# tomas-gr/RawNanoporeSignalCompression

Measured on AMD Instinct MI355X. Metric: MSamples/s encode+decode (1/2/4/8 GPU) at fixed ratio; % HBM roofline, higher is better.
Workload: dtype int16; 1 GPU; configs[1]: 100000 reads x 100000 int16 samples per GPU (1 chunk each), C5 encode+decode; reads_per_gpu=100000, samples_per_read=100000, global_reads=100000, parallelism=dp1 (reads round-robin, no data-path collective)

## Files before the change

rawnanoporesignalcompression_amd/csrc/model_capi.hip:

```cpp
#include <stdlib.h>
#include <string.h>

#define PGN_SELECT_HOST_ONLY
#include "pgn_segment.h"
#include "pgn_select.h"
#include "pgn_stitch.h"
#include "zstd1_dec.h"
#include "zstd1_model.h"

using namespace pgn::z1;

extern "C" {

size_t z1m_compress(const uint8_t* src, size_t n, uint8_t* dst, size_t cap)
{
    if (n > 0xFFFFFFF0ull || cap < compress_bound(n)) return 0;
    uint32_t* ht = (uint32_t*)calloc((size_t)1 << 15, 4);
    size_t ns = kMaxSrc / 4 + 2;
    Seq* seqs = (Seq*)malloc(ns * sizeof(Seq));
    uint8_t* codes = (uint8_t*)malloc(3 * ns);
    uint8_t* litbuf = (uint8_t*)malloc(kMaxSrc + 1);
    CompressWork* w = (CompressWork*)malloc(sizeof(CompressWork));
    size_t r = compress_serial(dst, src, n, ht, seqs, codes, codes + ns, codes + 2 * ns, litbuf, *w);
    free(w); free(litbuf); free(codes); free(seqs); free(ht);
// ... 140 lines not shown
    for (;; k++) {
        if (k % 64 == 0 && 2 * (k + 64) > maxKeys) { ok = 0; break; }
        const long pk = (long)e - 256;
        e += e >> 7;
        if (!(pk + 1 < ilimit)) break;
        const uint64_t v8 = rd64(src + pk);
        if (rd32(src + pk + 1) == (uint32_t)(v8 >> 16)) { ok = 0; break; }
        const uint32_t keys[2] = {(uint32_t)v8 ^ (hash_word(v8, p.hashLog, p.mls) * 0x9E3779B1u),
                                  (uint32_t)(v8 >> 8) ^ (hash_word(v8 >> 8, p.hashLog, p.mls) * 0x9E3779B1u)};
        for (int j = 0; j < 2 && ok; j++) {
            const uint32_t a = cert_fmix32(keys[j]), b = cert_fmix32(keys[j] ^ 0x5BD1E995u);
            const uint64_t m = (1ull << (a & 63u)) | (1ull << ((a >> 6) & 63u)) | (1ull << ((a >> 12) & 63u)) |
                               (1ull << ((a >> 18) & 63u)) | (1ull << ((a >> 24) & 63u)) | (1ull << (b & 63u));
            uint64_t* w = filt + ((b >> 6) & (words - 1));
            if ((*w & m) == m) ok = 0;
            *w |= m;
        }
        if (!ok) break;
    }
    free(filt);
    return ok;
}

long z1m_decompress(const uint8_t* src, size_t n, uint8_t* dst, size_t cap)
{
    DecWork* w = (DecWork*)malloc(sizeof(DecWork));
    long r = decompress_frames(src, n, dst, cap, *w);
    free(w);
    return r;
}

unsigned z1m_huf_lengths(const uint32_t* count, unsigned maxSymbolValue, uint8_t* nbBits)
{
    HufNode* nodes = (HufNode*)calloc(1024, sizeof(HufNode));
    huf_sort_serial(nodes + 1, count, maxSymbolValue);
    uint16_t val[256];
    const unsigned r = huf_build_from_sorted(nodes, maxSymbolValue, 11, nbBits, val);
    free(nodes);
    return r;
}

long long z1m_content_size(const uint8_t* src, size_t n)
{
    bool ok = false;
    uint64_t v = frame_content_size(src, n, &ok);
    return ok ? (long long)v : -1;
// ... 80 lines not shown
```

rawnanoporesignalcompression_amd/csrc/pgn_kernels.hip:

```cpp
#include <hip/hip_runtime.h>
#include <stdio.h>
#include <stdlib.h>
#include <string.h>

#include <algorithm>
#include <condition_variable>
#include <mutex>
#include <vector>

#include "../../include/pgnano_hip.h"
#include "../../include/pgnano_pod5.h"
#include "pgn_c5.h"
#include "pgn_internal.h"
#include "pgn_segment.h"
#include "pgn_stitch.h"
#include "pgn_ctc.h"
#include "pgn_crf.h"
#include "pgn_crf_post.h"
#include "pgn_qual.h"
#include "pgn_select.h"
#include "pgn_vbz.h"
#include "pgn_variants.h"
#include "pgn_zdec.h"
#include "pgn_zenc.h"
// ... 215 lines not shown
        sz[4] = tL;
    }
}

constexpr size_t kSplitWgMaxChunks = 64;

__global__ __launch_bounds__(64) __attribute__((amdgpu_waves_per_eu(4))) void enc_zstd_kernel(EncArgs a)
{
    const int lane = lane_id();
    const EncLayout lay = enc_layout();
    uint8_t* sbase = a.slotScratch + (size_t)blockIdx.x * a.slotBytes;
    EncScratch S;
    S.ht = (uint32_t*)(sbase + lay.ht);
    S.seqs = (z1::Seq*)(sbase + lay.seqs);
    S.codes = sbase + lay.codes;
    S.lit = sbase + lay.lit;
    S.seqSection = sbase + lay.seqSection;
    S.seqWork = (z1::SeqWork*)(sbase + lay.seqWork);
    S.maxSeq = kMaxEncSeq;
    S.huf = (uint32_t*)(sbase + lay.huf);
    S.coop = nullptr;
    uint32_t epoch = a.epochs[blockIdx.x];
    PhaseProf P;
    P.init(a.prof);
    const size_t G = a.G, units = (size_t)a.nu * G;
    while (true) {
        uint32_t u = 0;
        if (lane == 0) u = atomicAdd(a.queue, 1u);
        u = __builtin_amdgcn_readfirstlane(u);
        if (u >= units) break;
        const int s = a.nu == 1 ? 0 : unit_stream((uint32_t)(u / G));
        const size_t g = u % G;
        if (a.base + g >= a.nchunks) continue;
        const uint32_t n = a.sizes[g * kStreams + s];
        if (a.sizes[g * kStreams] == ~0u) continue;
        ht_next_epoch(S.ht, epoch, n);
        const uint8_t* src = a.streams + g * kChunkStreamBytes + (a.nu == 1 ? a.sizes[g * kStreams + 1] : stream_off(s));
        uint8_t* dst = a.frames + g * kChunkFrameBytes + frame_off(s);
        const size_t fsz = zstd1_compress_wave(dst, src, n, S, epoch & 0xFFu, P);
        if (lane == 0) a.fsizes[g * kStreams + s] = (uint32_t)fsz;
        wave_sync();
    }
    if (lane == 0) a.epochs[blockIdx.x] = epoch;
    P.flush();
}

__device__ __noinline__ void enc_place_frame(const EncArgs& a, size_t g, int s, const uint8_t* fr, uint32_t f)
// ... 42 lines not shown
    if (a.base + g >= a.nchunks) return;
    if (a.sizes[g * kStreams] == ~0u) return;
    __shared__ uint32_t winAll[(kCoopEncWaves - 1) * kWinWords];
    __shared__ CoopEncCmd cmdLds;
    lds_enc_cmd* cmd = (lds_enc_cmd*)&cmdLds;
    if (wid != 0) {
        coop_enc_helper_wave(wid, cmd, (lds_u32*)&winAll[(wid - 1) * kWinWords]);
        return;
    }
    const EncLayout lay = enc_layout();
    uint8_t* sbase = a.slotScratch + (size_t)u * a.slotBytes;
    EncScratch S;
    S.ht = (uint32_t*)(sbase + lay.ht);
    S.seqs = (z1::Seq*)(sbase + lay.seqs);
    S.codes = sbase + lay.codes;
    S.lit = sbase + lay.lit;
    S.seqSection = sbase + lay.seqSection;
    S.seqWork = (z1::SeqWork*)(sbase + lay.seqWork);
    S.maxSeq = kMaxEncSeq;
    S.huf = (uint32_t*)(sbase + lay.huf);
    S.coop = cmd;
    uint32_t epoch = a.epochs[u];
    PhaseProf P;
    P.init(a.prof);
    const uint32_t n = a.sizes[g * kStreams + s];
    ht_next_epoch(S.ht, epoch, n);
    const uint8_t* src = a.streams + g * kChunkStreamBytes + (a.nu == 1 ? a.sizes[g * kStreams + 1] : stream_off(s));
    uint8_t* dst = a.frames + g * kChunkFrameBytes + frame_off(s);
    const size_t fsz = zstd1_compress_wave<true>(dst, src, n, S, epoch & 0xFFu, P);
    if (lane == 0) {
        a.fsizes[g * kStreams + s] = (uint32_t)fsz;
        a.epochs[u] = epoch;
    }
    coop_enc_finish(cmd);
    if (a.lookback) enc_place_frame(a, g, s, dst, (uint32_t)fsz);
    P.flush();
}

__global__ __launch_bounds__(64) void enc_assemble_kernel(EncArgs a)
{
    const size_t g = blockIdx.x;
    const size_t c = a.base + g;
    if (g >= a.G || c >= a.nchunks) return;
    const int lane = lane_id();
    const uint32_t* sz = a.sizes + g * kStreams;
    if (sz[0] == ~0u) return;
    PhaseProf P;
// ... 998 lines not shown
template <int Codec>
__global__ __launch_bounds__(64) __attribute__((amdgpu_waves_per_eu(5))) void enc_chunk_kernel(EncArgs a)
{
    constexpr int nf = codec_frames(Codec);
    constexpr bool oneFrame = nf == 1;
    const int lane = lane_id();
    const EncLayout lay = enc_layout();
    uint8_t* sbase = a.slotScratch + (size_t)blockIdx.x * a.slotBytes;
    EncScratch S;
    S.ht = (uint32_t*)(sbase + lay.ht);
    S.seqs = (z1::Seq*)(sbase + lay.seqs);
    S.codes = sbase + lay.codes;
    S.lit = sbase + lay.lit;
    S.seqSection = sbase + lay.seqSection;
    S.seqWork = (z1::SeqWork*)(sbase + lay.seqWork);
    S.maxSeq = kMaxEncSeq;
    S.huf = (uint32_t*)(sbase + lay.huf);
    S.coop = nullptr;
    const uint32_t capN = a.capN;
    uint8_t* streams = sbase + lay.bytes;
    uint8_t* fbuf = streams + chunk_stream_bytes(capN);
    uint32_t epoch = a.epochs[blockIdx.x];
    PhaseProf P;
    P.init(a.prof);
    while (true) {
        uint32_t u = 0;
        if (lane == 0) u = atomicAdd(a.queue, 1u);
        u = __builtin_amdgcn_readfirstlane(u);
        if (u >= a.nchunks) break;
        const size_t c = a.list ? a.list[u] : u;
        const uint32_t n = a.sampleCounts[c];
        if (n > capN) {
            enc_fail_chunk(a, c, PGN_ERR_UNSUPPORTED);
            continue;
        }
        const int16_t* x = a.samples + a.sampleOffsets[c];
        uint32_t sz[kStreams] = {0, 0, 0, 0, 0};
        const uint8_t* src[kStreams] = {streams, streams, streams, streams, streams};
        if (Codec == kCodecVbz || Codec == kCodecC1) {
            const uint32_t pad = (16u - (svb_key_length(n) & 15u)) & 15u;
            const uint32_t m = vbz_split_chunk(x, n, streams + pad);
            src[0] = streams + pad;
            if (Codec == kCodecVbz) {
                sz[0] = m;
            } else {
                sz[0] = n ? svb_key_length(n) : 0u;
                sz[1] = m - sz[0];
// ... 2618 lines not shown
```

rawnanoporesignalcompression_amd/csrc/pgn_wave.h:

```cpp
#pragma once
#include <hip/hip_runtime.h>
#include <stdint.h>

namespace pgn {

constexpr size_t kCodecLdsBytes = 8192;
typedef __attribute__((address_space(3))) uint32_t lds_u32;
static __shared__ __attribute__((aligned(16))) uint8_t sCodecLds[kCodecLdsBytes];

constexpr int kWave = 64;

__device__ __forceinline__ int lane_id() { return (int)__lane_id(); }

__device__ __forceinline__ uint32_t readlane_u32(uint32_t v, int l)
{
    return (uint32_t)__builtin_amdgcn_readlane((int)v, l);
}
__device__ __forceinline__ uint64_t readlane_u64(uint64_t v, int l)
{
    uint32_t lo = readlane_u32((uint32_t)v, l), hi = readlane_u32((uint32_t)(v >> 32), l);
    return ((uint64_t)hi << 32) | lo;
}
__device__ __forceinline__ uint64_t ballot(bool p) { return __ballot(p); }

// ... 154 lines not shown
        gst<uint4>(dst + i + 3072, d);
    }
    for (; i + 16 <= n; i += 1024) gst<uint4>(dst + i, gld<uint4>(src + i));
    for (size_t b = (n & ~(size_t)15) + (size_t)lane; b < n; b += 64) gst<uint8_t>(dst + b, gb(src + b));
}
__device__ inline void wave_copy8(uint8_t* dst, const uint8_t* src, size_t n)
{
    const size_t l16 = (size_t)lane_id() * 16;
    size_t base = 0;
    for (; base + 8192 <= n; base += 8192) {
        uint4 v[8];
#pragma unroll
        for (int k = 0; k < 8; k++) v[k] = gld<uint4>(src + base + l16 + 1024 * k);
#pragma unroll
        for (int k = 0; k < 8; k++) gst<uint4>(dst + base + l16 + 1024 * k, v[k]);
    }
    wave_copy(dst + base, src + base, n - base);
}
__device__ inline void wave_fill(uint8_t* dst, uint8_t v, size_t n)
{
    for (size_t i = lane_id(); i < n; i += 64) gst<uint8_t>(dst + i, v);
}

constexpr int kPhases = 16;
constexpr int kCounters = 16;
constexpr int kHufProfOff = 2 * (kPhases + kCounters);
constexpr int kProfWords = kHufProfOff + 2 * (kPhases + kCounters);
struct PhaseProf {
#ifdef PGN_PROFILE
    uint64_t* out;
    uint64_t last;
    uint64_t acc[kPhases];
    uint64_t cnt[kCounters];
    __device__ void init(uint64_t* o)
    {
        out = o;
        for (int i = 0; i < kPhases; i++) acc[i] = 0;
        for (int i = 0; i < kCounters; i++) cnt[i] = 0;
        last = o ? __builtin_amdgcn_s_memtime() : 0;
    }
    __device__ __forceinline__ void mark(int phase)
    {
        if (out) {
            uint64_t t = __builtin_amdgcn_s_memtime();
            acc[phase] += t - last;
            last = t;
        }
    }
    __device__ __forceinline__ void count(int k, uint64_t v = 1)
    {
        if (out) cnt[k] += v;
    }
    __device__ void flush()
    {
        if (out && lane_id() == 0) {
            for (int i = 0; i < kPhases; i++) atomicAdd((unsigned long long*)&out[i], (unsigned long long)acc[i]);
            for (int i = 0; i < kCounters; i++)
                atomicAdd((unsigned long long*)&out[2 * kPhases + i], (unsigned long long)cnt[i]);
        }
    }
#else
    __device__ __forceinline__ void init(uint64_t*) {}
    __device__ __forceinline__ void mark(int) {}
    __device__ __forceinline__ void count(int, uint64_t = 1) {}
    __device__ __forceinline__ void flush() {}
#endif
};

}
```

rawnanoporesignalcompression_amd/csrc/pgn_zenc.h:

```cpp
#pragma once
#ifndef PGN_AB_SKIP
#define PGN_AB_SKIP 0
#endif
#include "pgn_c5.h"
#include "pgn_wave.h"
#include "zstd1_model.h"

namespace pgn {

constexpr int kWinWords = 392;
constexpr int kFiltSlots = 512;

struct WCTable {
    uint32_t tableLog;
    uint16_t stateTable[64];
    uint32_t deltaNbBits[16];
    int32_t deltaFindState[16];
};

struct alignas(16) EncLds {
    union {
        struct {
            uint64_t filt[kFiltSlots];
            uint32_t vh0[64], vh1[64], vpk[64];
            uint32_t vd0[64], vd1[64];
        };
        struct {
            uint32_t hist2[2][256];
            union {
            uint32_t hist2x[1 + 2 * 256];
            struct {
            uint8_t nbBits[256];
            uint16_t val[256];
            union {
// ... 166 lines not shown
constexpr uint32_t kCertWords = kCodecLdsBytes / 8;
constexpr uint32_t kCertKeys = 2048;
__device__ __forceinline__ uint32_t fmix32(uint32_t x)
{
    x ^= x >> 16;
    x *= 0x85EBCA6Bu;
    x ^= x >> 13;
    x *= 0xC2B2AE35u;
    x ^= x >> 16;
    return x;
}
typedef __attribute__((address_space(3))) uint64_t lds_u64;
__device__ __forceinline__ bool cert_insert(lds_u64* words, uint32_t x)
{
    const uint32_t a = fmix32(x), b = fmix32(x ^ 0x5BD1E995u);
    const uint64_t m = (1ull << (a & 63u)) | (1ull << ((a >> 6) & 63u)) | (1ull << ((a >> 12) & 63u)) |
                       (1ull << ((a >> 18) & 63u)) | (1ull << ((a >> 24) & 63u)) | (1ull << (b & 63u));
    const uint32_t w = (b >> 6) & (kCertWords - 1u);
    const uint64_t old = __hip_atomic_fetch_or(words + w, m, __ATOMIC_RELAXED, __HIP_MEMORY_SCOPE_WORKGROUP);
    return (old & m) == m;
}
static_assert((kCertWords & (kCertWords - 1)) == 0, "filter words: a power of two");
__device__ __noinline__ bool no_match_certificate(const uint8_t* __restrict__ src, uint32_t n, unsigned hlog, unsigned mls,
                                                  uint32_t off1)
{
    const uint32_t lane = (uint32_t)lane_id();
    src = uni(src);
    n = uni(n);
    hlog = uni(hlog);
    mls = uni(mls);
    off1 = uni(off1);
    lds_u64* words = (lds_u64*)sCodecLds;
    for (uint32_t i = lane; i < kCertWords; i += 64) words[i] = 0;
    lds_sync();
    const int32_t ilimit = (int32_t)n - 8;
    const uint32_t* E = kVisitChains.e[1];
    auto loads = [&](int32_t p, uint64_t& v, uint32_t& r) {
        if (p + 1 < ilimit) {
            v = ld64u(src + p);
            r = off1 > 0 ? ld32u(src + p + 2 - (int32_t)off1) : 0u;
        }
    };
    int32_t pk = (int32_t)E[lane] - 256, pkN = (int32_t)E[64 + lane] - 256;
    uint64_t v8 = 0;
    uint32_t rw = 0;
    loads(pk, v8, rw);
    for (uint32_t ci = 0;; ci += 64) {
        if (2 * (ci + 64) > kCertKeys) return false;
        uint64_t v8N = 0;
        uint32_t rwN = 0;
        loads(pkN, v8N, rwN);
        const int32_t pkNN = (int32_t)E[ci + 128 + lane] - 256;
        const bool valid = pk + 1 < ilimit;
        bool bad = false;
        if (valid) {
            bad = off1 > 0 && rw == (uint32_t)(v8 >> 16);
            const uint32_t h0 = z1::hash_word(v8, hlog, mls), h1 = z1::hash_word(v8 >> 8, hlog, mls);
            if (cert_insert(words, (uint32_t)v8 ^ (h0 * 0x9E3779B1u))) bad = true;
            if (cert_insert(words, (uint32_t)(v8 >> 8) ^ (h1 * 0x9E3779B1u))) bad = true;
        }
        if (ballot(bad)) return false;
        if (ballot(!valid)) return true;
        pk = pkN;
        pkN = pkNN;
        v8 = v8N;
        rw = rwN;
    }
}

struct SearchOut {
    uint32_t nbSeq, lastLL, rep0, rep1, rounds;
    uint32_t candIters;
};
__device__ __noinline__ SearchOut fast_search_wave(const uint8_t* __restrict__ src, uint32_t start, uint32_t end, unsigned hlog,
                                                   unsigned mls, uint32_t* __restrict__ ht, uint32_t tag,
                                                   z1::Seq* __restrict__ seqs, uint32_t rep0, uint32_t rep1, uint32_t idxBits,
                                                   uint32_t lowIdx, uint32_t maxRep, bool single)
{
    EncLds& L = sEnc;
    const uint32_t lane = (uint32_t)lane_id();
    src = uni(src);
    start = uni(start);
    end = uni(end);
    hlog = uni(hlog);
#ifdef PGN_AB_HLOG
    hlog = hlog > PGN_AB_HLOG ? PGN_AB_HLOG : hlog;
#endif
    mls = uni(mls);
    ht = uni(ht);
    tag = uni(tag);
    seqs = uni(seqs);
    rep0 = uni(rep0);
    rep1 = uni(rep1);
    idxBits = uni(idxBits);
    const uint32_t idxMask = (1u << idxBits) - 1u, fpMask = ((1u << kTagShift) - 1u) & ~idxMask;
    const int32_t iend = (int32_t)end, ilimit = (int32_t)end - 8;
    int32_t ip0 = (int32_t)start + (start == 0 ? 1 : 0), anchor = (int32_t)start;
    lowIdx = uni(lowIdx);
    maxRep = uni(maxRep);
    single = __builtin_amdgcn_readfirstlane((int)single) != 0;
    uint32_t off1 = rep0, off2 = rep1, offSaved = 0;
    if (off2 > maxRep) { offSaved = off2; off2 = 0; }
    if (off1 > maxRep) { offSaved = off1; off1 = 0; }
#ifdef PGN_NO_CERT
    single = false;
#endif
    if (single && no_match_certificate(src, end, hlog, mls, off1)) {
        SearchOut r;
        r.nbSeq = 0;
        r.lastLL = end - start;
        r.rep0 = off1 ? off1 : offSaved;
        r.rep1 = off2 ? off2 : offSaved;
        r.rounds = 0;
        r.candIters = 0;
        return r;
    }
    uint32_t nbSeq = 0, rounds = 0, candIters = 0;
    const uint64_t below = (1ull << lane) - 1ull, above = ~below & ~(1ull << lane);
    for (int i = (int)lane; i < kFiltSlots; i += 64) L.filt[i] = 0;
    lds_sync();
    uint32_t chain = (start == 0) ? 1u : 0u, ci = 0;
    auto positions = [&](uint32_t c, int32_t& pkOut, int32_t& pNextOut) {
        const uint32_t* E = kVisitChains.e[chain];
        pkOut = (int32_t)E[c + lane] + (anchor - 256);
        pNextOut = (int32_t)E[c + 64] + (anchor - 256);
    };
    int32_t pk = 0, pNext = 0;
    uint64_t v8 = 0;
    uint32_t repw = 0;
    auto loads = [&](int32_t p, uint64_t& v, uint32_t& r) {
        if (p + 1 < ilimit) {
            v = ld64u(src + p);
            r = (off1 > 0) ? ld32u(src + p + 2 - (int32_t)off1) : 0u;
        }
    };
    bool havePk = false;
    while (ip0 + 1 < ilimit) {
// ... 199 lines not shown
                    off1 = t;
                    if (lane == 0) {
                        const uint64_t wr = ld64u(src + ip0);
                        gst<uint32_t>(ht + z1::hash_word(wr, hlog, mls), ht_entry(tag, (uint32_t)ip0 + 1, (uint32_t)wr, idxBits));
                        seqs[nbSeq].litLength = 0;
                        seqs[nbSeq].offset = 1;
                        seqs[nbSeq].mlBase = rLength - 3;
                    }
                    nbSeq++;
                    ip0 += (int32_t)rLength;
                    anchor = ip0;
                }
            }
        }
        wave_sync();
    }
    SearchOut r;
    r.nbSeq = nbSeq;
    r.lastLL = (uint32_t)(iend - anchor);
    r.rep0 = off1 ? off1 : offSaved;
    r.rep1 = off2 ? off2 : offSaved;
    r.rounds = rounds;
    r.candIters = candIters;
    return r;
}

__device__ __noinline__ void huf_encode_segment_wave(uint8_t* __restrict__ out, const uint8_t* __restrict__ src, uint32_t len,
                                                     uint32_t totalBits, lds_u32* win)
{
    const uint32_t lane = (uint32_t)lane_id();
    out = uni(out);
    src = uni(src);
    len = uni(len);
    totalBits = uni(totalBits);
    const uint32_t* cw = sEnc.cw;
    for (uint32_t w = lane; w < (uint32_t)kWinWords; w += 64) win[w] = 0;
    lds_sync();
    uint32_t winLo = 0;
    uint32_t bitBase = 0;
    uint4 nv = make_uint4(0, 0, 0, 0);
    if ((int32_t)len - 16 - (int32_t)(16 * lane) >= 0) nv = gld<uint4>(src + (len - 16 - 16 * lane));
    auto step = [&](auto FULL, uint32_t r0) {
        const int32_t a = (int32_t)len - 16 - (int32_t)(r0 + 16 * lane);
        uint32_t wv[4];
        if (FULL || a >= 0) {
            const uint4 v = nv;
// ... 1338 lines not shown
    const size_t h = z1::frame_header_size(n, n < 7 ? 10u : z1::level1_params(n).windowLog);
    if (n < 7) {
        if (lane == 0) z1::write_raw_block_frame(dst, src, n);
        return h + 3 + n;
    }
    const z1::Params p = z1::level1_params(n);
    P.count(12);
    if (lane == 0) z1::write_frame_header(dst, n, p.windowLog);
    size_t o = h;
    uint32_t rep0 = 1, rep1 = 4;
    uint32_t hufCur = 0, hufCheck = 0;
    for (uint32_t start = 0; start < n; start += (uint32_t)z1::kMaxSrc) {
        const uint32_t bs = (n - start < (uint32_t)z1::kMaxSrc) ? n - start : (uint32_t)z1::kMaxSrc;
        const bool last = start + bs == n, first = start == 0;
        uint8_t* bdst = dst + o;
        uint32_t cSize = 0;
        size_t seqSize = 0;
#if PGN_AB_SKIP == 1
        if (false) {
#else
        if (bs >= 7) {
#endif
            const uint32_t ip0 = start + (start == 0 ? 1u : 0u);
            const SearchOut so = fast_search_wave(src, start, start + bs, p.hashLog, p.mls, S.ht, tag, S.seqs, rep0, rep1,
                                                  ht_idx_bits(n), z1::window_low_index(start + bs, p.windowLog),
                                                  ip0 + 1u - z1::window_low_index(ip0, p.windowLog), first && last);
            const uint32_t nbSeq = uni(so.nbSeq), lastLL = uni(so.lastLL);
            P.mark(1);
            P.count(0, uni(so.rounds));
            P.count(14, uni(so.candIters));
            P.count(1, nbSeq);
            P.count(13);
#if PGN_AB_SKIP == 2
            if (uni(so.nbSeq) < 0x7FFFFFFFu) goto raw_block;
#endif
            const uint8_t* lit = src + start;
            uint32_t nLit = bs;
            if (nbSeq > 0) {
                uint32_t pos = start, q = 0;
                for (uint32_t i = 0; i < nbSeq; i++) {
                    const z1::Seq sq = S.seqs[i];
                    wave_copy(S.lit + q, src + pos, sq.litLength);
                    q += sq.litLength;
                    pos += sq.litLength + sq.mlBase + 3;
                }
                wave_copy(S.lit + q, src + pos, lastLL);
                q += lastLL;
                wave_sync();
                lit = S.lit;
                nLit = q;
// ... 59 lines not shown
```

rawnanoporesignalcompression_amd/csrc/zstd1_model.h:

```cpp
#pragma once
#include "zstd1_common.h"

namespace pgn {
namespace z1 {

PGN_HD size_t match_count(const uint8_t* src, size_t a, size_t b, size_t end)
{
    size_t n = 0;
    while (a + n < end && src[a + n] == src[b + n]) n++;
    return n;
}

PGN_HD size_t fast_search_serial(const uint8_t* src, size_t start, size_t end, const Params& p, uint32_t* ht,
                                 uint32_t rep[3], Seq* seqs, size_t* lastLL)
{
    const unsigned hlog = p.hashLog, mls = p.mls;
    size_t nbSeq = 0;
    long ip0 = (long)start + (start == 0 ? 1 : 0), anchor = (long)start;
    long ip1 = ip0 + 1;
    const long iend = (long)end, ilimit = (long)end - 8;
    const uint32_t lowIdx = window_low_index(end, p.windowLog);
    const long prefixStart = (long)lowIdx - 1;
    uint32_t offset_1 = rep[0], offset_2 = rep[1], offsetSaved = 0;
    {
// ... 57 lines not shown
            ht[hash_at(src + ip0 - 2, hlog, mls)] = (uint32_t)(ip0 - 2) + 1;
            if (offset_2 > 0) {
                while ((ip0 <= ilimit) && (rd32(src + ip0) == rd32(src + ip0 - offset_2))) {
                    size_t rLength = match_count(src, (size_t)ip0 + 4, (size_t)ip0 + 4 - offset_2, (size_t)iend) + 4;
                    uint32_t t = offset_2; offset_2 = offset_1; offset_1 = t;
                    ht[hash_at(src + ip0, hlog, mls)] = (uint32_t)ip0 + 1;
                    ip0 += (long)rLength;
                    seqs[nbSeq].litLength = 0;
                    seqs[nbSeq].offset = 1;
                    seqs[nbSeq].mlBase = (uint32_t)(rLength - 3);
                    nbSeq++;
                    anchor = ip0;
                }
            }
        }
        ip1 = ip0 + 1;
    }
    rep[0] = offset_1 ? offset_1 : offsetSaved;
    rep[1] = offset_2 ? offset_2 : offsetSaved;
    *lastLL = (size_t)(iend - anchor);
    return nbSeq;
}

struct HufState {
    uint8_t nbBits[256];
    uint16_t val[256];
    bool check;
};

struct LitWork {
    uint32_t count[256];
    HufNode nodes[2 * 256 + 1];
    uint8_t nbBits[256];
    uint16_t val[256];
    FseCTable fct;
    uint8_t scratch[64];
};

PGN_HD size_t write_raw_literals(uint8_t* dst, const uint8_t* lit, size_t n)
{
    size_t fl = write_rawrle_lit_header(dst, n, kSetBasic);
    for (size_t i = 0; i < n; i++) dst[fl + i] = lit[i];
    return fl + n;
}

PGN_HD size_t huf_encode_1x(uint8_t* dst, const uint8_t* src, size_t n, const uint8_t* nbBits, const uint16_t* val)
// ... 291 lines not shown
```

Measured before the change: 241,600 MSamples/s.

## Add LDS-resident small-block match search with bloom filter and log

Adds a wave-level search path for small blocks that stages the block in LDS and replaces the global hash table with a per-block bloom filter plus an append-only log of hashed positions. A serial reference version and a C API entry are added for checking it. The aim is to avoid hash-table epoch maintenance and global-memory probes for small inputs. The path falls back to the regular search when the log overflows, and it adds extra LDS synchronisation and per-candidate log scans.

```diff
diff --git a/rawnanoporesignalcompression_amd/csrc/model_capi.hip b/rawnanoporesignalcompression_amd/csrc/model_capi.hip
--- a/rawnanoporesignalcompression_amd/csrc/model_capi.hip
+++ b/rawnanoporesignalcompression_amd/csrc/model_capi.hip
@@ -186,6 +186,40 @@
     return ok;
 }
 
+size_t z1m_small_search(const uint8_t* src, size_t n, int mode, uint32_t* out3, size_t maxSeq, uint32_t* info)
+{
+    if (n < 7 || n > kMaxSrc) return (size_t)-1;
+    const Params p = level1_params(n);
+    Seq* seqs = (Seq*)malloc((n / 4 + 2) * sizeof(Seq));
+    size_t lastLL = 0, nb = (size_t)-1;
+    uint32_t rep[3] = {1, 4, 8};
+    for (int i = 0; i < 15; i++) info[i] = 0;
+    if (mode == 1 && n <= kSmallSearchBytes) {
+        SmallSearchWork* w = (SmallSearchWork*)malloc(sizeof(SmallSearchWork));
+        SmallSearchInfo si;
+        nb = small_search_serial(src, n, p, rep, seqs, &lastLL, *w, &si);
+        free(w);
+        info[0] = nb != (size_t)-1;
+        info[1] = nb == (size_t)-1;
+        info[6] = si.rounds; info[7] = si.logEntries; info[8] = si.flagged; info[9] = si.falsePositives; info[10] = si.scans;
+        info[11] = si.refutedAbsent; info[12] = si.shadowed; info[13] = si.fpThenHit; info[14] = si.repFirst;
+    }
+    if (nb == (size_t)-1) {
+        uint32_t* ht = (uint32_t*)calloc((size_t)1 << 15, 4);
+        rep[0] = 1; rep[1] = 4;
+        nb = fast_search_serial(src, 0, n, p, ht, rep, seqs, &lastLL);
+        free(ht);
+    }
+    info[2] = (uint32_t)nb; info[3] = (uint32_t)lastLL; info[4] = rep[0]; info[5] = rep[1];
+    for (size_t i = 0; i < nb && i < maxSeq; i++) {
+        out3[3 * i] = seqs[i].litLength; out3[3 * i + 1] = seqs[i].offset; out3[3 * i + 2] = seqs[i].mlBase;
+    }
+    free(seqs);
+    return nb;
+}
+unsigned z1m_small_search_bytes(void) { return kSmallSearchBytes; }
+unsigned z1m_small_search_log_cap(void) { return kSmallLogCap; }
+
 long z1m_decompress(const uint8_t* src, size_t n, uint8_t* dst, size_t cap)
 {
     DecWork* w = (DecWork*)malloc(sizeof(DecWork));
diff --git a/rawnanoporesignalcompression_amd/csrc/pgn_kernels.hip b/rawnanoporesignalcompression_amd/csrc/pgn_kernels.hip
--- a/rawnanoporesignalcompression_amd/csrc/pgn_kernels.hip
+++ b/rawnanoporesignalcompression_amd/csrc/pgn_kernels.hip
@@ -261,7 +261,7 @@
     S.coop = nullptr;
     uint32_t epoch = a.epochs[blockIdx.x];
     PhaseProf P;
-    P.init(a.prof);
+    P.init(a.prof, a.prof);
     const size_t G = a.G, units = (size_t)a.nu * G;
     while (true) {
         uint32_t u = 0;
@@ -350,7 +350,7 @@
     S.coop = cmd;
     uint32_t epoch = a.epochs[u];
     PhaseProf P;
-    P.init(a.prof);
+    P.init(a.prof, a.prof);
     const uint32_t n = a.sizes[g * kStreams + s];
     ht_next_epoch(S.ht, epoch, n);
     const uint8_t* src = a.streams + g * kChunkStreamBytes + (a.nu == 1 ? a.sizes[g * kStreams + 1] : stream_off(s));
@@ -1395,7 +1395,7 @@
     uint8_t* fbuf = streams + chunk_stream_bytes(capN);
     uint32_t epoch = a.epochs[blockIdx.x];
     PhaseProf P;
-    P.init(a.prof);
+    P.init(a.prof, a.prof);
     while (true) {
         uint32_t u = 0;
         if (lane == 0) u = atomicAdd(a.queue, 1u);
diff --git a/rawnanoporesignalcompression_amd/csrc/pgn_wave.h b/rawnanoporesignalcompression_amd/csrc/pgn_wave.h
--- a/rawnanoporesignalcompression_amd/csrc/pgn_wave.h
+++ b/rawnanoporesignalcompression_amd/csrc/pgn_wave.h
@@ -200,21 +200,29 @@
     for (size_t i = lane_id(); i < n; i += 64) gst<uint8_t>(dst + i, v);
 }
 
+#ifdef PGN_PROFILE
+#define PGN_PROF(...) __VA_ARGS__
+#else
+#define PGN_PROF(...)
+#endif
 constexpr int kPhases = 16;
 constexpr int kCounters = 16;
 constexpr int kHufProfOff = 2 * (kPhases + kCounters);
 constexpr int kProfWords = kHufProfOff + 2 * (kPhases + kCounters);
+static_assert(kHufProfOff + 2 * kPhases <= kProfWords, "PhaseProf::ext's words lie inside the profile buffer");
 struct PhaseProf {
 #ifdef PGN_PROFILE
     uint64_t* out;
     uint64_t last;
     uint64_t acc[kPhases];
     uint64_t cnt[kCounters];
-    __device__ void init(uint64_t* o)
+    __device__ void init(uint64_t* o, uint64_t* extBase = nullptr)
     {
         out = o;
+        extOut = o ? extBase : nullptr;
         for (int i = 0; i < kPhases; i++) acc[i] = 0;
         for (int i = 0; i < kCounters; i++) cnt[i] = 0;
+        for (int i = 0; i < kPhases; i++) extv[i] = 0;
         last = o ? __builtin_amdgcn_s_memtime() : 0;
     }
     __device__ __forceinline__ void mark(int phase)
@@ -229,18 +237,28 @@
     {
         if (out) cnt[k] += v;
     }
+    uint64_t* extOut;
+    uint64_t extv[kPhases];
+    __device__ __forceinline__ void ext(int k, uint64_t v)
+    {
+        if (extOut) extv[k] += v;
+    }
     __device__ void flush()
     {
         if (out && lane_id() == 0) {
+            if (extOut)
+                for (int i = 0; i < kPhases; i++)
+                    atomicAdd((unsigned long long*)&extOut[kHufProfOff + kPhases + i], (unsigned long long)extv[i]);
             for (int i = 0; i < kPhases; i++) atomicAdd((unsigned long long*)&out[i], (unsigned long long)acc[i]);
             for (int i = 0; i < kCounters; i++)
                 atomicAdd((unsigned long long*)&out[2 * kPhases + i], (unsigned long long)cnt[i]);
         }
     }
 #else
-    __device__ __forceinline__ void init(uint64_t*) {}
+    __device__ __forceinline__ void init(uint64_t*, uint64_t* = nullptr) {}
     __device__ __forceinline__ void mark(int) {}
     __device__ __forceinline__ void count(int, uint64_t = 1) {}
+    __device__ __forceinline__ void ext(int, uint64_t) {}
     __device__ __forceinline__ void flush() {}
 #endif
 };
diff --git a/rawnanoporesignalcompression_amd/csrc/pgn_zenc.h b/rawnanoporesignalcompression_amd/csrc/pgn_zenc.h
--- a/rawnanoporesignalcompression_amd/csrc/pgn_zenc.h
+++ b/rawnanoporesignalcompression_amd/csrc/pgn_zenc.h
@@ -10,6 +10,7 @@
 
 constexpr int kWinWords = 392;
 constexpr int kFiltSlots = 512;
+using z1::kSmallSearchBytes;
 
 struct WCTable {
     uint32_t tableLog;
@@ -222,7 +223,7 @@
 }
 static_assert((kCertWords & (kCertWords - 1)) == 0, "filter words: a power of two");
 __device__ __noinline__ bool no_match_certificate(const uint8_t* __restrict__ src, uint32_t n, unsigned hlog, unsigned mls,
-                                                  uint32_t off1)
+                                                  uint32_t off1 PGN_PROF(, uint32_t* certRounds = nullptr))
 {
     const uint32_t lane = (uint32_t)lane_id();
     src = uni(src);
@@ -247,6 +248,9 @@
     loads(pk, v8, rw);
     for (uint32_t ci = 0;; ci += 64) {
         if (2 * (ci + 64) > kCertKeys) return false;
+#ifdef PGN_PROFILE
+        if (certRounds) ++*certRounds;
+#endif
         uint64_t v8N = 0;
         uint32_t rwN = 0;
         loads(pkN, v8N, rwN);
@@ -271,7 +275,345 @@
 struct SearchOut {
     uint32_t nbSeq, lastLL, rep0, rep1, rounds;
     uint32_t candIters;
+    PGN_PROF(uint32_t certRounds, certCycles;)
+    PGN_PROF(uint32_t smallPath;)
 };
+
+constexpr int kSmallFiltSlots = 128;
+constexpr uint32_t kSmallBlkWords = z1::kSmallSearchBytes / 4 + 4;
+constexpr uint32_t kSmallOverflow = 0xFFFFFFFFu;
+struct alignas(16) SmallLds {
+    uint64_t filt[kSmallFiltSlots];
+    uint32_t vh0[64], vh1[64], vpk[64], vd0[64], vd1[64];
+    uint64_t bloom[z1::kSmallBloomWords];
+    uint32_t log[z1::kSmallLogCap];
+    uint32_t blk[kSmallBlkWords];
+};
+static_assert(sizeof(SmallLds) <= kCodecLdsBytes, "small-block search LDS exceeds the codec LDS");
+static_assert(z1::kSmallSearchBytes + 1 < (1u << 16), "log entries hold the index in 16 bits");
+static_assert(z1::kSmallSearchBytes <= (1u << 15), "log entries hold the hash (hashLog <= 16) in 16 bits");
+#define sSmall (*reinterpret_cast<SmallLds*>(sCodecLds))
+__device__ __forceinline__ uint32_t sblk_ld32(const SmallLds& L, int32_t p)
+{
+    const uint32_t w = (uint32_t)p >> 2, sh = 8u * ((uint32_t)p & 3u);
+    return (uint32_t)((((uint64_t)L.blk[w + 1] << 32) | L.blk[w]) >> sh);
+}
+__device__ __forceinline__ uint64_t sblk_ld64(const SmallLds& L, int32_t p)
+{
+    const uint32_t w = (uint32_t)p >> 2, sh = 8u * ((uint32_t)p & 3u);
+    const uint32_t a = L.blk[w], b = L.blk[w + 1], c = L.blk[w + 2];
+    const uint32_t lo = (uint32_t)((((uint64_t)b << 32) | a) >> sh), hi = (uint32_t)((((uint64_t)c << 32) | b) >> sh);
+    return ((uint64_t)hi << 32) | lo;
+}
+__device__ __forceinline__ uint32_t sblk_byte(const SmallLds& L, int32_t p)
+{
+    return (L.blk[(uint32_t)p >> 2] >> (8u * ((uint32_t)p & 3u))) & 0xFFu;
+}
+__device__ inline uint32_t sblk_match_count(const SmallLds& L, uint32_t a, uint32_t b, uint32_t end)
+{
+    const uint32_t o = 4u * (uint32_t)lane_id();
+    uint32_t n = 0;
+    while (a + n < end) {
+        const uint32_t len = end - (a + n);
+        const uint32_t nv = len > o ? (len - o < 4u ? len - o : 4u) : 0u;
+        uint32_t x = 0;
+        if (nv) {
+            x = sblk_ld32(L, (int32_t)(a + n + o)) ^ sblk_ld32(L, (int32_t)(b + n + o));
+            if (nv < 4u) x &= (1u << (8u * nv)) - 1u;
+        }
+        const uint32_t mism = x ? o + ((uint32_t)__builtin_ctz(x) >> 3) : 0xFFFFFFFFu;
+        const uint64_t mm = ballot(mism != 0xFFFFFFFFu);
+        if (mm) return n + readlane_u32(mism, __builtin_ctzll(mm));
+        if (len <= 256u) return len + n;
+        n += 256;
+    }
+    return n;
+}
+__device__ inline uint32_t sblk_back_count(const SmallLds& L, uint32_t a, uint32_t b, uint32_t lim)
+{
+    const uint32_t lane = (uint32_t)lane_id();
+    uint32_t n = 0;
+    while (n < lim) {
+        const uint32_t o = n + lane + 1;
+        const bool diff = (o <= lim) && sblk_byte(L, (int32_t)(a - o)) != sblk_byte(L, (int32_t)(b - o));
+        const uint64_t m = ballot(diff || o > lim);
+        if (m) return n + (uint32_t)__builtin_ctzll(m);
+        n += 64;
+    }
+    return lim;
+}
+__device__ __noinline__ SearchOut small_search_wave(const uint8_t* __restrict__ src, uint32_t n, unsigned hlog, unsigned mls,
+                                                    z1::Seq* __restrict__ seqs, uint32_t rep0, uint32_t rep1)
+{
+    SmallLds& L = sSmall;
+    const uint32_t lane = (uint32_t)lane_id();
+    src = uni(src);
+    n = uni(n);
+    hlog = uni(hlog);
+    mls = uni(mls);
+    seqs = uni(seqs);
+    uint32_t off1 = uni(rep0), off2 = uni(rep1), offSaved = 0;
+    if (off2 > 1) { offSaved = off2; off2 = 0; }
+    if (off1 > 1) { offSaved = off1; off1 = 0; }
+    const int32_t iend = (int32_t)n, ilimit = (int32_t)n - 8;
+    const uint32_t lowIdx = 1;
+    SearchOut r;
+    r.candIters = 0;
+    PGN_PROF(r.certRounds = 0;)
+    PGN_PROF(const uint64_t certT0 = __builtin_amdgcn_s_memtime();)
+#if !defined(PGN_NO_CERT) && !defined(PGN_SMALL_NO_CERT)
+    const bool certified = no_match_certificate(src, n, hlog, mls, off1 PGN_PROF(, &r.certRounds));
+#else
+    const bool certified = false;
+#endif
+    PGN_PROF(r.certCycles = (uint32_t)(__builtin_amdgcn_s_memtime() - certT0);)
+    if (certified) {
+        r.nbSeq = 0;
+        r.lastLL = n;
+        r.rep0 = off1 ? off1 : offSaved;
+        r.rep1 = off2 ? off2 : offSaved;
+        r.rounds = 0;
+        PGN_PROF(r.smallPath = 0;)
+        return r;
+    }
+    PGN_PROF(r.smallPath = 2;)
+    r.nbSeq = kSmallOverflow;
+    r.lastLL = r.rep0 = r.rep1 = r.rounds = 0;
+    for (uint32_t w = lane; w < (n + 3) / 4 + 4; w += 64) {
+        uint32_t x = 0;
+        if (4 * w + 4 <= n) x = ld32u(src + 4 * w);
+        else
+            for (uint32_t b = 0; b < 4; b++)
+                if (4 * w + b < n) x |= (uint32_t)gb(src + 4 * w + b) << (8 * b);
+        L.blk[w] = x;
+    }
+    for (uint32_t i = lane; i < (uint32_t)kSmallFiltSlots; i += 64) L.filt[i] = 0;
+    for (uint32_t i = lane; i < z1::kSmallBloomWords; i += 64) L.bloom[i] = 0;
+    lds_sync();
+    uint32_t nbSeq = 0, rounds = 0, logN = 0;
+    const uint64_t below = (1ull << lane) - 1ull;
+    int32_t ip0 = 1, anchor = 0;
+    uint32_t chain = 1, ci = 0;
+    auto insert = [&](int32_t pos) {
+        const uint64_t w = uni(sblk_ld64(L, pos));
+        const uint32_t h = z1::hash_word(w, hlog, mls);
+        uint32_t bw;
+        const uint64_t bm = z1::small_bloom_bits(h, (uint32_t)w, &bw);
+        if (lane == 0) {
+            L.log[logN] = (h << 16) | ((uint32_t)pos + 1);
+            L.bloom[bw] |= bm;
+        }
+        logN++;
+    };
+    while (ip0 + 1 < ilimit) {
+        rounds++;
+        const uint32_t* E = kVisitChains.e[chain];
+        const int32_t pk = (int32_t)E[ci + lane] + (anchor - 256), pNext = (int32_t)E[ci + 64] + (anchor - 256);
+        const bool valid = (pk + 1 < ilimit);
+        uint64_t v8 = 0;
+        uint32_t repw = 0;
+        if (valid) {
+            v8 = sblk_ld64(L, pk);
+            repw = (off1 > 0) ? sblk_ld32(L, pk + 2 - (int32_t)off1) : 0u;
+        }
+        const bool rep = valid && (off1 > 0) && (repw == (uint32_t)(v8 >> 16));
+        const uint64_t repb = ballot(rep);
+        int f = 64;
+        bool repf = false, c0f = false;
+        uint32_t m0f = 0, m1f = 0, fwdKnown = 0;
+        if (repb & 1) {
+            if (logN + 2 > z1::kSmallLogCap) return r;
+            insert(ip0);
+            insert(ip0 + 1);
+            f = 0;
+            repf = true;
+        } else {
+        uint32_t h0 = 0xFFFFFFFFu, h1 = 0xFFFFFFFEu;
+        uint64_t M0 = 0, M1 = 0, bm0 = 0, bm1 = 0;
+        uint32_t bw0 = 0, bw1 = 0;
+        bool maybe0 = false, maybe1 = false;
+        if (valid) {
+            h0 = z1::hash_word(v8, hlog, mls);
+            h1 = z1::hash_word(v8 >> 8, hlog, mls);
+            bm0 = z1::small_bloom_bits(h0, (uint32_t)v8, &bw0);
+            bm1 = z1::small_bloom_bits(h1, (uint32_t)(v8 >> 8), &bw1);
+            maybe0 = (L.bloom[bw0] & bm0) == bm0;
+            maybe1 = (L.bloom[bw1] & bm1) == bm1;
+            atomicOr((unsigned long long*)&L.filt[h0 & (kSmallFiltSlots - 1)], (unsigned long long)(1ull << lane));
+            atomicOr((unsigned long long*)&L.filt[h1 & (kSmallFiltSlots - 1)], (unsigned long long)(1ull << lane));
+        }
+        L.vh0[lane] = h0;
+        L.vh1[lane] = h1;
+        L.vpk[lane] = (uint32_t)pk;
+        L.vd0[lane] = (uint32_t)v8;
+        L.vd1[lane] = (uint32_t)(v8 >> 8);
+        lds_sync();
+        if (valid) {
+            M0 = L.filt[h0 & (kSmallFiltSlots - 1)];
+            M1 = L.filt[h1 & (kSmallFiltSlots - 1)];
+            atomicOr((unsigned long long*)&L.bloom[bw0], (unsigned long long)bm0);
+            atomicOr((unsigned long long*)&L.bloom[bw1], (unsigned long long)bm1);
+        }
+        lds_sync();
+        if (valid) {
+            L.filt[h0 & (kSmallFiltSlots - 1)] = 0;
+            L.filt[h1 & (kSmallFiltSlots - 1)] = 0;
+        }
+        uint32_t m0 = 0, m1 = 0, d0 = 0, d1 = 0;
+        bool fw0 = false, fw1 = false;
+        for (uint64_t cand = M0 & below; cand;) {
+            const int jj = 63 - __builtin_clzll(cand);
+            const uint32_t pj = L.vpk[jj];
+            if (L.vh1[jj] == h0) { m0 = pj + 2; d0 = L.vd1[jj]; fw0 = true; break; }
+            if (L.vh0[jj] == h0) { m0 = pj + 1; d0 = L.vd0[jj]; fw0 = true; break; }
+            cand &= ~(1ull << jj);
+        }
+        for (uint64_t cand = M1 & below; cand;) {
+            const int jj = 63 - __builtin_clzll(cand);
+            const uint32_t pj = L.vpk[jj];
+            if (L.vh1[jj] == h1) { m1 = pj + 2; d1 = L.vd1[jj]; fw1 = true; break; }
+            if (L.vh0[jj] == h1) { m1 = pj + 1; d1 = L.vd0[jj]; fw1 = true; break; }
+            cand &= ~(1ull << jj);
+        }
+        bool c0 = false, c1 = false;
+        if (valid) {
+            c0 = fw0 ? (m0 > lowIdx && d0 == (uint32_t)v8) : maybe0;
+            c1 = fw1 ? (m1 > lowIdx && d1 == (uint32_t)(v8 >> 8)) : maybe1;
+        }
+        uint64_t hits = ballot(rep || c0 || c1);
+        {
+            const uint64_t fwb0 = ballot(fw0), fwb1 = ballot(fw1);
+            while (hits) {
+                const int ff = __builtin_ctzll(hits);
+                if ((repb >> ff) & 1) break;
+                const bool isC0 = (ballot(c0) >> ff) & 1;
+                if (((isC0 ? fwb0 : fwb1) >> ff) & 1) break;
+                const uint32_t hq = readlane_u32(isC0 ? h0 : h1, ff);
+                uint32_t mf = 0;
+                for (int32_t base = (int32_t)logN; base > 0; base -= 64) {
+                    const int32_t i = base - 1 - (int32_t)lane;
+                    const uint32_t e = i >= 0 ? L.log[i] : 0u;
+                    const uint64_t mm = ballot(i >= 0 && (e >> 16) == hq);
+                    if (mm) {
+                        mf = readlane_u32(e, __builtin_ctzll(mm)) & 0xFFFFu;
+                        break;
+                    }
+                }
+                const uint32_t ipc = readlane_u32((uint32_t)pk, ff) + (isC0 ? 0u : 1u);
+                const uint32_t nm = mf > lowIdx ? sblk_match_count(L, ipc, mf - 1, (uint32_t)iend) : 0u;
+                if (nm >= 4) {
+                    if ((int)lane == ff) {
+                        if (isC0) m0 = mf;
+                        else m1 = mf;
+                    }
+                    fwdKnown = nm;
+                    break;
+                }
+                if ((int)lane == ff) {
+                    if (isC0) c0 = false;
+                    else c1 = false;
+                }
+                hits = ballot(rep || c0 || c1);
+            }
+        }
+        const uint64_t vmask = ballot(valid);
+        f = hits ? __builtin_ctzll(hits) : 64;
+        const int lastCommit = hits ? f : (63 - __builtin_clzll(vmask));
+        {
+            const uint64_t cm = ballot(valid && (int)lane <= lastCommit);
+            const uint32_t cnt = 2u * (uint32_t)__builtin_popcountll(cm);
+            if (logN + cnt > z1::kSmallLogCap) return r;
+            if ((cm >> lane) & 1) {
+                const uint32_t at = logN + 2u * mbcnt(cm);
+                L.log[at] = (h0 << 16) | ((uint32_t)pk + 1);
+                L.log[at + 1] = (h1 << 16) | ((uint32_t)pk + 2);
+            }
+            logN += cnt;
+        }
+        lds_sync();
+        if (!hits) {
+            if (vmask == ~0ull) {
+                ip0 = pNext;
+                ci += 64;
+                continue;
+            }
+            break;
+        }
+        repf = (repb >> f) & 1;
+        c0f = (ballot(c0) >> f) & 1;
+        m0f = readlane_u32(m0, f);
+        m1f = readlane_u32(m1, f);
+        }
+        const int32_t ipf = (int32_t)readlane_u32((uint32_t)pk, f);
+        const uint32_t cur0 = (uint32_t)ipf + 1;
+        int32_t ipm, match0;
+        uint32_t mLength, offcode;
+        if (repf) {
+            const int32_t ip2 = ipf + 2;
+            mLength = (sblk_byte(L, ip2 - 1) == sblk_byte(L, ip2 - (int32_t)off1 - 1)) ? 1u : 0u;
+            ipm = ip2 - (int32_t)mLength;
+            match0 = ipm - (int32_t)off1;
+            mLength += 4;
+            offcode = 0;
+        } else {
+            if (c0f) { ipm = ipf; match0 = (int32_t)m0f - 1; }
+            else { ipm = ipf + 1; match0 = (int32_t)m1f - 1; }
+            off2 = off1;
+            off1 = (uint32_t)(ipm - match0);
+            offcode = off1 + 2;
+            mLength = 4;
+            const int32_t lim = (ipm - anchor) < match0 ? (ipm - anchor) : match0;
+            const uint32_t back = lim > 0 ? sblk_back_count(L, (uint32_t)ipm, (uint32_t)match0, (uint32_t)lim) : 0u;
+            ipm -= (int32_t)back;
+            match0 -= (int32_t)back;
+            mLength += back;
+        }
+        mLength += fwdKnown ? fwdKnown - 4u
+                            : sblk_match_count(L, (uint32_t)ipm + mLength, (uint32_t)match0 + mLength, (uint32_t)iend);
+        if (lane == 0) {
+            seqs[nbSeq].litLength = (uint32_t)(ipm - anchor);
+            seqs[nbSeq].offset = offcode + 1;
+            seqs[nbSeq].mlBase = mLength - 3;
+        }
+        nbSeq++;
+        ip0 = ipm + (int32_t)mLength;
+        anchor = ip0;
+        chain = 0;
+        ci = 0;
+        if (ip0 <= ilimit) {
+            if (logN + 2 > z1::kSmallLogCap) return r;
+            insert((int32_t)cur0 + 1);
+            insert(ip0 - 2);
+            if (off2 > 0) {
+                while ((ip0 <= ilimit) && sblk_ld32(L, ip0) == sblk_ld32(L, ip0 - (int32_t)off2)) {
+                    const uint32_t rLength = sblk_match_count(L, (uint32_t)ip0 + 4, (uint32_t)ip0 + 4 - off2, (uint32_t)iend) + 4;
+                    const uint32_t t = off2;
+                    off2 = off1;
+                    off1 = t;
+                    if (logN + 1 > z1::kSmallLogCap) return r;
+                    insert(ip0);
+                    if (lane == 0) {
+                        seqs[nbSeq].litLength = 0;
+                        seqs[nbSeq].offset = 1;
+                        seqs[nbSeq].mlBase = rLength - 3;
+                    }
+                    nbSeq++;
+                    ip0 += (int32_t)rLength;
+                    anchor = ip0;
+                }
+            }
+        }
+        lds_sync();
+    }
+    PGN_PROF(r.smallPath = 1;)
+    r.nbSeq = nbSeq;
+    r.lastLL = (uint32_t)(iend - anchor);
+    r.rep0 = off1 ? off1 : offSaved;
+    r.rep1 = off2 ? off2 : offSaved;
+    r.rounds = rounds;
+    return r;
+}
+
 __device__ __noinline__ SearchOut fast_search_wave(const uint8_t* __restrict__ src, uint32_t start, uint32_t end, unsigned hlog,
                                                    unsigned mls, uint32_t* __restrict__ ht, uint32_t tag,
                                                    z1::Seq* __restrict__ seqs, uint32_t rep0, uint32_t rep1, uint32_t idxBits,
@@ -305,14 +647,25 @@
 #ifdef PGN_NO_CERT
     single = false;
 #endif
-    if (single && no_match_certificate(src, end, hlog, mls, off1)) {
+#ifdef PGN_PROFILE
+    uint32_t certRounds = 0;
+    const uint64_t certT0 = __builtin_amdgcn_s_memtime();
+    const bool certified = single && no_match_certificate(src, end, hlog, mls, off1, &certRounds);
+    const uint32_t certCycles = (uint32_t)(__builtin_amdgcn_s_memtime() - certT0);
+#else
+    const bool certified = single && no_match_certificate(src, end, hlog, mls, off1);
+#endif
+    if (certified) {
         SearchOut r;
+        PGN_PROF(r.certRounds = certRounds;)
+        PGN_PROF(r.certCycles = certCycles;)
         r.nbSeq = 0;
         r.lastLL = end - start;
         r.rep0 = off1 ? off1 : offSaved;
         r.rep1 = off2 ? off2 : offSaved;
         r.rounds = 0;
         r.candIters = 0;
+        PGN_PROF(r.smallPath = 0;)
         return r;
     }
     uint32_t nbSeq = 0, rounds = 0, candIters = 0;
@@ -558,6 +911,9 @@
     r.rep1 = off2 ? off2 : offSaved;
     r.rounds = rounds;
     r.candIters = candIters;
+    PGN_PROF(r.certRounds = certRounds;)
+    PGN_PROF(r.certCycles = certCycles;)
+    PGN_PROF(r.smallPath = 0;)
     return r;
 }
 
@@ -1942,10 +2298,35 @@
         if (bs >= 7) {
 #endif
             const uint32_t ip0 = start + (start == 0 ? 1u : 0u);
-            const SearchOut so = fast_search_wave(src, start, start + bs, p.hashLog, p.mls, S.ht, tag, S.seqs, rep0, rep1,
-                                                  ht_idx_bits(n), z1::window_low_index(start + bs, p.windowLog),
-                                                  ip0 + 1u - z1::window_low_index(ip0, p.windowLog), first && last);
+            SearchOut so;
+            so.nbSeq = kSmallOverflow;
+            bool again = false;
+#ifndef PGN_NO_SMALL_SEARCH
+            if (first && last && bs <= kSmallSearchBytes) {
+                so = small_search_wave(src, bs, p.hashLog, p.mls, S.seqs, rep0, rep1);
+                again = true;
+            }
+#endif
+            if (uni(so.nbSeq) == kSmallOverflow) {
+                so = fast_search_wave(src, start, start + bs, p.hashLog, p.mls, S.ht, tag, S.seqs, rep0, rep1, ht_idx_bits(n),
+                                      z1::window_low_index(start + bs, p.windowLog),
+                                      ip0 + 1u - z1::window_low_index(ip0, p.windowLog), first && last && !again);
+                PGN_PROF(if (again) so.smallPath = 2;)
+            }
             const uint32_t nbSeq = uni(so.nbSeq), lastLL = uni(so.lastLL);
+#ifdef PGN_PROFILE
+            if (P.out) {
+                const int k = (first && last && bs <= kSmallSearchBytes) ? 0 : 6;
+                P.ext(k + 5, __builtin_amdgcn_s_memtime() - P.last);
+                P.ext(k, 1);
+                P.ext(k + 1, uni(so.certRounds));
+                P.ext(k + 2, uni(so.certCycles));
+                P.ext(k + 3, uni(so.rounds));
+                P.ext(k + 4, uni(so.rounds) ? 1 : 0);
+                P.ext(12, uni(so.smallPath) == 1 ? 1 : 0);
+                P.ext(13, uni(so.smallPath) == 2 ? 1 : 0);
+            }
+#endif
             P.mark(1);
             P.count(0, uni(so.rounds));
             P.count(14, uni(so.candIters));
diff --git a/rawnanoporesignalcompression_amd/csrc/zstd1_model.h b/rawnanoporesignalcompression_amd/csrc/zstd1_model.h
--- a/rawnanoporesignalcompression_amd/csrc/zstd1_model.h
+++ b/rawnanoporesignalcompression_amd/csrc/zstd1_model.h
@@ -103,6 +103,226 @@
     return nbSeq;
 }
 
+constexpr uint32_t kSmallSearchBytes = 2048;
+constexpr uint32_t kSmallLogCap = 688;
+constexpr uint32_t kSmallBloomWords = 128;
+struct SmallSearchWork {
+    uint32_t log[kSmallLogCap];
+    uint64_t bloom[kSmallBloomWords];
+};
+struct SmallSearchInfo {
+    uint32_t rounds, logEntries, flagged, falsePositives, scans;
+    uint32_t refutedAbsent;
+    uint32_t shadowed;
+    uint32_t fpThenHit;
+    uint32_t repFirst;
+};
+PGN_HD uint32_t small_fmix32(uint32_t x)
+{
+    x ^= x >> 16;
+    x *= 0x85EBCA6Bu;
+    x ^= x >> 13;
+    x *= 0xC2B2AE35u;
+    x ^= x >> 16;
+    return x;
+}
+PGN_HD uint64_t small_bloom_bits(uint32_t h, uint32_t v, uint32_t* word)
+{
+    const uint32_t a = small_fmix32(v ^ (h * 0x9E3779B1u));
+    *word = (a >> 24) & (kSmallBloomWords - 1u);
+    return (1ull << (a & 63u)) | (1ull << ((a >> 6) & 63u)) | (1ull << ((a >> 12) & 63u)) | (1ull << ((a >> 18) & 63u));
+}
+PGN_HD size_t small_search_serial(const uint8_t* src, size_t n, const Params& p, uint32_t rep[3], Seq* seqs, size_t* lastLL,
+                                  SmallSearchWork& W, SmallSearchInfo* info)
+{
+    const unsigned hlog = p.hashLog, mls = p.mls;
+    const long iend = (long)n, ilimit = (long)n - 8;
+    const uint32_t lowIdx = 1;
+    size_t nbSeq = 0;
+    long anchor = 0;
+    uint32_t off1 = rep[0], off2 = rep[1], offSaved = 0;
+    if (off2 > 1) { offSaved = off2; off2 = 0; }
+    if (off1 > 1) { offSaved = off1; off1 = 0; }
+    uint32_t logN = 0;
+    for (uint32_t i = 0; i < kSmallBloomWords; i++) W.bloom[i] = 0;
+    SmallSearchInfo I = {0, 0, 0, 0, 0, 0, 0, 0, 0};
+    bool overflow = false;
+    auto bloom_add = [&](uint32_t h, uint32_t v) {
+        uint32_t w;
+        const uint64_t m = small_bloom_bits(h, v, &w);
+        W.bloom[w] |= m;
+    };
+    auto bloom_has = [&](uint32_t h, uint32_t v) {
+        uint32_t w;
+        const uint64_t m = small_bloom_bits(h, v, &w);
+        return (W.bloom[w] & m) == m;
+    };
+    auto log_add = [&](uint32_t h, uint32_t idx) {
+        if (logN >= kSmallLogCap) { overflow = true; return; }
+        W.log[logN++] = (h << 16) | idx;
+    };
+    auto log_latest = [&](uint32_t h) -> uint32_t {
+        for (uint32_t i = logN; i > 0; i--)
+            if ((W.log[i - 1] >> 16) == h) return W.log[i - 1] & 0xFFFFu;
+        return 0;
+    };
+    uint32_t e0 = 257;
+    long ip0 = 1;
+    while (ip0 + 1 < ilimit && !overflow) {
+        I.rounds++;
+        long pk[64];
+        uint32_t h0[64], h1[64], v0[64], v1[64], m0[64], m1[64];
+        bool valid[64], repk[64], c0[64], c1[64], fw0[64], fw1[64];
+        uint32_t e = e0;
+        int nValid = 0;
+        for (int k = 0; k < 64; k++) {
+            pk[k] = (long)e - 256 + anchor;
+            e += e >> 7;
+            valid[k] = pk[k] + 1 < ilimit;
+            repk[k] = c0[k] = c1[k] = fw0[k] = fw1[k] = false;
+            m0[k] = m1[k] = 0;
+            if (!valid[k]) continue;
+            nValid = k + 1;
+            const uint64_t v8 = rd64(src + pk[k]);
+            h0[k] = hash_word(v8, hlog, mls);
+            h1[k] = hash_word(v8 >> 8, hlog, mls);
+            v0[k] = (uint32_t)v8;
+            v1[k] = (uint32_t)(v8 >> 8);
+            repk[k] = off1 > 0 && rd32(src + pk[k] + 2 - (long)off1) == (uint32_t)(v8 >> 16);
+            if (k == 0 && repk[0]) {
+                I.repFirst++;
+                break;
+            }
+            uint32_t d0 = 0, d1 = 0;
+            for (int j = k - 1; j >= 0 && !fw0[k]; j--) {
+                if (h1[j] == h0[k]) { m0[k] = (uint32_t)pk[j] + 2; d0 = v1[j]; fw0[k] = true; }
+                else if (h0[j] == h0[k]) { m0[k] = (uint32_t)pk[j] + 1; d0 = v0[j]; fw0[k] = true; }
+            }
+            for (int j = k - 1; j >= 0 && !fw1[k]; j--) {
+                if (h1[j] == h1[k]) { m1[k] = (uint32_t)pk[j] + 2; d1 = v1[j]; fw1[k] = true; }
+                else if (h0[j] == h1[k]) { m1[k] = (uint32_t)pk[j] + 1; d1 = v0[j]; fw1[k] = true; }
+            }
+            c0[k] = fw0[k] ? (m0[k] > lowIdx && d0 == v0[k]) : bloom_has(h0[k], v0[k]);
+            c1[k] = fw1[k] ? (m1[k] > lowIdx && d1 == v1[k]) : bloom_has(h1[k], v1[k]);
+            if (!fw0[k] && c0[k]) I.flagged++;
+            if (!fw1[k] && c1[k]) I.flagged++;
+        }
+        for (int k = 0; k < nValid; k++) {
+            bloom_add(h0[k], v0[k]);
+            bloom_add(h1[k], v1[k]);
+        }
+        int f = 64;
+        uint32_t fwdKnown = 0;
+        bool dropped = false;
+        for (int k = 0; k < nValid && f == 64; k++) {
+            while (repk[k] || c0[k] || c1[k]) {
+                if (repk[k]) { f = k; break; }
+                const bool isC0 = c0[k];
+                if (isC0 ? fw0[k] : fw1[k]) { f = k; break; }
+                I.scans++;
+                const uint32_t mf = log_latest(isC0 ? h0[k] : h1[k]);
+                const size_t nm = mf > lowIdx ? match_count(src, (size_t)pk[k] + (isC0 ? 0 : 1), mf - 1, (size_t)iend) : 0;
+                if (nm >= 4) {
+                    (isC0 ? m0[k] : m1[k]) = mf;
+                    fwdKnown = (uint32_t)nm;
+                    f = k;
+                    break;
+                }
+                I.falsePositives++;
+                dropped = true;
+                if (mf == 0) I.refutedAbsent++;
+                else {
+                    const uint32_t hq = isC0 ? h0[k] : h1[k], vq = isC0 ? v0[k] : v1[k];
+                    bool older = false;
+                    for (uint32_t i = 0; i < logN; i++)
+                        if ((W.log[i] >> 16) == hq && rd32(src + (W.log[i] & 0xFFFFu) - 1) == vq) older = true;
+                    if (older) I.shadowed++;
+                }
+                if (isC0) c0[k] = false;
+                else c1[k] = false;
+            }
+        }
+        if (dropped && f < 64) I.fpThenHit++;
+        const int lastCommit = f < 64 ? f : nValid - 1;
+        for (int k = 0; k <= lastCommit; k++) {
+            log_add(h0[k], (uint32_t)pk[k] + 1);
+            log_add(h1[k], (uint32_t)pk[k] + 2);
+        }
+        if (overflow) break;
+        if (f == 64) {
+            if (nValid < 64) break;
+            ip0 = (long)e - 256 + anchor;
+            e0 = e;
+            continue;
+        }
+        const long ipf = pk[f];
+        const uint32_t cur0 = (uint32_t)ipf + 1;
+        long ipm, match0;
+        size_t mLength;
+        uint32_t offcode;
+        if (repk[f]) {
+            const long ip2 = ipf + 2;
+            mLength = (src[ip2 - 1] == src[ip2 - (long)off1 - 1]) ? 1 : 0;
+            ipm = ip2 - (long)mLength;
+            match0 = ipm - (long)off1;
+            mLength += 4;
+            offcode = 0;
+        } else {
+            if (c0[f]) { ipm = ipf; match0 = (long)m0[f] - 1; }
+            else { ipm = ipf + 1; match0 = (long)m1[f] - 1; }
+            off2 = off1;
+            off1 = (uint32_t)(ipm - match0);
+            offcode = off1 + 2;
+            mLength = 4;
+            while (ipm > anchor && match0 > 0 && src[ipm - 1] == src[match0 - 1]) {
+                ipm--;
+                match0--;
+                mLength++;
+            }
+        }
+        mLength += fwdKnown ? fwdKnown - 4 : match_count(src, (size_t)ipm + mLength, (size_t)match0 + mLength, (size_t)iend);
+        seqs[nbSeq].litLength = (uint32_t)(ipm - anchor);
+        seqs[nbSeq].offset = offcode + 1;
+        seqs[nbSeq].mlBase = (uint32_t)(mLength - 3);
+        nbSeq++;
+        ip0 = ipm + (long)mLength;
+        anchor = ip0;
+        e0 = 256;
+        if (ip0 <= ilimit) {
+            auto insert = [&](long pos) {
+                const uint64_t w = rd64(src + pos);
+                const uint32_t h = hash_word(w, hlog, mls);
+                log_add(h, (uint32_t)pos + 1);
+                bloom_add(h, (uint32_t)w);
+            };
+            insert((long)cur0 + 1);
+            insert(ip0 - 2);
+            if (off2 > 0) {
+                while (ip0 <= ilimit && rd32(src + ip0) == rd32(src + ip0 - (long)off2)) {
+                    const size_t rLength = match_count(src, (size_t)ip0 + 4, (size_t)ip0 + 4 - off2, (size_t)iend) + 4;
+                    const uint32_t t = off2;
+                    off2 = off1;
+                    off1 = t;
+                    insert(ip0);
+                    ip0 += (long)rLength;
+                    seqs[nbSeq].litLength = 0;
+                    seqs[nbSeq].offset = 1;
+                    seqs[nbSeq].mlBase = (uint32_t)(rLength - 3);
+                    nbSeq++;
+                    anchor = ip0;
+                }
+            }
+        }
+    }
+    I.logEntries = logN;
+    if (info) *info = I;
+    if (overflow) return (size_t)-1;
+    rep[0] = off1 ? off1 : offSaved;
+    rep[1] = off2 ? off2 : offSaved;
+    *lastLL = (size_t)(iend - anchor);
+    return nbSeq;
+}
+
 struct HufState {
     uint8_t nbBits[256];
     uint16_t val[256];
```

Measured after the change: 244,900 MSamples/s, median of 6. 1.4% higher.
